# fugue-project/fugue

Hardware: NVIDIA H100
Metric: transform() rows/sec, hash-partitioned (num=256) identity map, 8-col table (higher is better)
Workload: dtype int64+f64 (byte moves; u64 hash arithmetic)

## Files before the change

### fugue_b200/csrc/fb_partition.cu

```cuda
#include <stdlib.h>

#include <mutex>

#include "fb_common.cuh"

namespace {

constexpr int kBlock = 512;
constexpr int kItems = 8;
constexpr int kTile = kBlock * kItems;
constexpr int kWarps = kBlock / 32;
constexpr int kCtasPerSm = 2;

struct FbCols {
  const void* src[FB_MAX_COLS];
  void* dst[FB_MAX_COLS];
  int32_t width[FB_MAX_COLS];
  int32_t ncols;
};

struct ChunkGeom {
  int64_t nrows;
  int64_t full_rows;
  int64_t tiles_per_chunk;
// ... 287 lines not shown
  while (c < cols.ncols) {
    T* __restrict__ buf = (T*)(cx.buf + (size_t)(phase & 1) * kTile);
#pragma unroll
    for (int r = 0; r < kItems; ++r) buf[pos[r]] = v[r];
    int nxt = c + 1;
    while (nxt < cols.ncols && cols.width[nxt] != (int)sizeof(T)) ++nxt;
    if (nxt < cols.ncols) load_col<T, kFull>(cols.src[nxt], warp_row0, warp_rows, lane, v);
    __syncthreads();
    T* __restrict__ out = (T*)cols.dst[c];
#pragma unroll
    for (int k = 0; k < kItems; ++k) {
      const int j = k * kBlock + (int)threadIdx.x;
      if (kFull || j < tile_rows) out[dst[k]] = buf[j];
    }
    ++phase;
    c = nxt;
  }
}

template <bool kSingleU64, int kBits, bool kFull, bool kAll8>
__device__ __forceinline__ void scatter_tile(const FbKeys& keys, const FbDiv& dv, const uint32_t num,
                                             const FbCols& cols, const TileCtx& cx,
                                             const int64_t tile_row0, const int tile_rows, int& phase) {
  const unsigned lane = threadIdx.x & 31, warp = threadIdx.x >> 5;
  const unsigned lt = fb_lanemask_lt();
  const uint32_t nb = num + 1;
  const uint32_t nbp = cx.nbp;
  uint32_t* __restrict__ my_cnt = cx.cnt + warp * nbp;
  const int64_t warp_row0 = tile_row0 + (int64_t)warp * (32 * kItems);
  const int warp_rows = tile_rows - (int)warp * (32 * kItems);

  uint32_t pid[kItems];
#pragma unroll
  for (int r = 0; r < kItems; ++r) {
    const bool ok = kFull || (r * 32 + (int)lane) < warp_rows;
    pid[r] = ok ? compute_pid<kSingleU64>(keys, dv, warp_row0 + r * 32 + lane) : num;
  }

  uint32_t pos[kItems];
#pragma unroll
  for (int r = 0; r < kItems; ++r) {
    const unsigned m = match_lanes<kBits + (kFull ? 0 : 1)>(pid[r], 0xFFFFFFFFu);
    const unsigned before = __popc(m & lt);
    uint32_t old = 0;
    if (before == 0) {
      old = my_cnt[pid[r]];
      my_cnt[pid[r]] = old + __popc(m);
    }
    __syncwarp();
    old = __shfl_sync(0xFFFFFFFFu, old, __ffs(m) - 1);
    pos[r] = old + before;
  }
  __syncthreads();

  {
    const uint32_t per = (nb + kBlock - 1) / kBlock;
    const uint32_t b0 = threadIdx.x * per;
    uint32_t tot[kMaxPer];
    uint32_t sum = 0;
#pragma unroll
    for (int i = 0; i < kMaxPer; ++i) {
      tot[i] = 0;
      if ((uint32_t)i < per && b0 + i < nb) {
        uint32_t run = 0;
#pragma unroll
        for (int w = 0; w < kWarps; ++w) {
          const uint32_t t = cx.cnt[w * nbp + b0 + i];
          cx.cnt[w * nbp + b0 + i] = run;
          run += t;
        }
        tot[i] = run;
        sum += run;
      }
    }
    uint32_t x = sum;
#pragma unroll
    for (int o = 1; o < 32; o <<= 1) {
      const uint32_t y = __shfl_up_sync(0xFFFFFFFFu, x, o);
      if (lane >= (unsigned)o) x += y;
    }
    if (lane == 31) cx.scanw[warp] = x;
    __syncthreads();
    uint32_t run = x - sum;
    {
      const uint32_t wt = lane < kWarps ? cx.scanw[lane] : 0;
#pragma unroll
      for (int w = 0; w < kWarps; ++w) {
        const uint32_t v = __shfl_sync(0xFFFFFFFFu, wt, w);
        if ((unsigned)w < warp) run += v;
      }
    }
#pragma unroll
    for (int i = 0; i < kMaxPer; ++i) {
      if ((uint32_t)i < per && b0 + i < nb) {
        const uint32_t cur = cx.cursor[b0 + i];
        cx.bin_start[b0 + i] = run;
        cx.delta[b0 + i] = cur - run;
        cx.cursor[b0 + i] = cur + tot[i];
        run += tot[i];
      }
    }
  }
  __syncthreads();

#pragma unroll
  for (int r = 0; r < kItems; ++r) {
    pos[r] += cx.bin_start[pid[r]] + my_cnt[pid[r]];
    cx.pid_sorted[pos[r]] = (uint16_t)pid[r];
  }
  __syncthreads();
  uint32_t dst[kItems];
#pragma unroll
  for (int k = 0; k < kItems; ++k) {
    const int j = k * kBlock + (int)threadIdx.x;
    dst[k] = cx.delta[cx.pid_sorted[j]] + (uint32_t)j;
  }
  for (uint32_t i = threadIdx.x; i < (uint32_t)kWarps * nbp; i += kBlock) cx.cnt[i] = 0;

  move_columns<uint64_t, kFull>(cols, cx, pos, dst, warp_row0, warp_rows, tile_rows, lane, phase);
  if (!kAll8) {
    move_columns<uint32_t, kFull>(cols, cx, pos, dst, warp_row0, warp_rows, tile_rows, lane, phase);
    move_columns<uint16_t, kFull>(cols, cx, pos, dst, warp_row0, warp_rows, tile_rows, lane, phase);
    move_columns<uint8_t, kFull>(cols, cx, pos, dst, warp_row0, warp_rows, tile_rows, lane, phase);
  }
  __syncthreads();
}

template <bool kSingleU64, int kBits, bool kAll8>
__global__ void __launch_bounds__(kBlock, kCtasPerSm)
fb_scatter_kernel(FbKeys keys, FbDiv dv, uint32_t num, ChunkGeom g, int chunk0,
                  const uint32_t* __restrict__ chunk_base, const int64_t* __restrict__ part_offsets,
                  FbCols cols) {
  extern __shared__ __align__(128) uint64_t smem64[];
  TileCtx cx;
  cx.nbp = nb_padded(num);
  cx.buf = smem64;
  cx.delta = (uint32_t*)(smem64 + 2 * kTile);
  cx.cursor = cx.delta + cx.nbp;
  cx.bin_start = cx.cursor + cx.nbp;
  cx.cnt = cx.bin_start + cx.nbp;
  cx.scanw = cx.cnt + kWarps * cx.nbp;
  cx.pid_sorted = (uint16_t*)(cx.scanw + 32);

  const int chunk = chunk0 + (int)blockIdx.x;
  int64_t chunk_row0, chunk_row1;
  chunk_range(g, chunk, chunk_row0, chunk_row1);

  for (uint32_t b = threadIdx.x; b < cx.nbp; b += kBlock)
    cx.cursor[b] = b < num ? (uint32_t)part_offsets[b] + chunk_base[(size_t)chunk * num + b] : 0u;
  for (uint32_t i = threadIdx.x; i < (uint32_t)kWarps * cx.nbp; i += kBlock) cx.cnt[i] = 0;
  __syncthreads();

  int phase = 0;
  for (int64_t tile_row0 = chunk_row0; tile_row0 < chunk_row1; tile_row0 += kTile) {
    const int64_t left = chunk_row1 - tile_row0;
    if (left >= kTile)
      scatter_tile<kSingleU64, kBits, true, kAll8>(keys, dv, num, cols, cx, tile_row0, kTile, phase);
    else
      scatter_tile<kSingleU64, kBits, false, kAll8>(keys, dv, num, cols, cx, tile_row0, (int)left, phase);
  }
}

constexpr int kSwcMaxCols = 8;
constexpr uint32_t kSwcMaxNum = 256;

__device__ __forceinline__ uint32_t smem_u32(const void* p) { return (uint32_t)__cvta_generic_to_shared(p); }

__device__ __forceinline__ void mbar_init(uint32_t bar, uint32_t count) {
  asm volatile("mbarrier.init.shared::cta.b64 [%0], %1;" ::"r"(bar), "r"(count) : "memory");
}
__device__ __forceinline__ void mbar_expect_tx(uint32_t bar, uint32_t bytes) {
  asm volatile("mbarrier.arrive.expect_tx.shared::cta.b64 _, [%0], %1;" ::"r"(bar), "r"(bytes) : "memory");
}
__device__ __forceinline__ void mbar_arrive_relaxed(uint32_t bar) {
  asm volatile("mbarrier.arrive.relaxed.cta.shared::cta.b64 _, [%0];" ::"r"(bar) : "memory");
}
__device__ __forceinline__ void mbar_wait(uint32_t bar, uint32_t parity) {
  asm volatile(
      "{\n"
      ".reg .pred p;\n"
      "FB_WAIT:\n"
      "mbarrier.try_wait.parity.shared::cta.b64 p, [%0], %1;\n"
      "@p bra FB_DONE;\n"
      "bra FB_WAIT;\n"
      "FB_DONE:\n"
      "}\n" ::"r"(bar), "r"(parity)
      : "memory");
}
__device__ __forceinline__ uint64_t l2_policy_evict_normal() {
  uint64_t pol;
  asm volatile("createpolicy.fractional.L2::evict_normal.b64 %0, 1.0;" : "=l"(pol));
  return pol;
}
__device__ __forceinline__ uint64_t l2_policy_evict_last() {
  uint64_t pol;
  asm volatile("createpolicy.fractional.L2::evict_last.b64 %0, 1.0;" : "=l"(pol));
  return pol;
}
__device__ __forceinline__ void tma_load_1d(uint32_t dst_smem, const void* src, uint32_t bytes, uint32_t bar,
                                            uint64_t policy) {
  asm volatile(
      "cp.async.bulk.shared::cluster.global.mbarrier::complete_tx::bytes.L2::cache_hint [%0], [%1], %2, [%3], %4;"
      ::"r"(dst_smem), "l"(src), "r"(bytes), "r"(bar), "l"(policy)
      : "memory");
}

constexpr int kWsMoverWarps = 16, kWsRankWarps = 8;
constexpr int kWsMovers = kWsMoverWarps * 32, kWsRankers = kWsRankWarps * 32;
constexpr int kWsThreads = kWsMovers + kWsRankers + 128;
constexpr int kWsG = 16;
constexpr int kWsGWide = 4;
constexpr int kWsMinStages = 3;
constexpr int kWsRankItems = 16;
constexpr uint32_t kWsProducerRegs = 24, kWsRankerRegs = 64, kWsMoverRegs = 88;
static_assert(128 * kWsProducerRegs + kWsRankers * kWsRankerRegs + kWsMovers * kWsMoverRegs <= kWsThreads * 72,
              "setmaxnreg: the roles take more registers than the launch gives the CTA");
constexpr int kMoveBatch = 8;

struct WsUnits {
  const uint64_t* src[FB_MAX_COLS];
  uint64_t* dst[FB_MAX_COLS];
  int32_t nunits;
  int32_t per_group;
  int32_t ngroups;
};

__device__ __forceinline__ void ws_chunk_run(const ChunkGeom& g, int i, int S, int& c0, int64_t& r0, int64_t& r1) {
  c0 = (int)((int64_t)i * g.nchunks_full / S);
  const int c1 = (int)((int64_t)(i + 1) * g.nchunks_full / S);
  int64_t unused;
  chunk_range(g, c0, r0, unused);
  chunk_range(g, c1 - 1, unused, r1);
}

struct WsMap {
  const uint64_t* src2[FB_MAX_COLS];
  uint64_t a[FB_MAX_COLS], b[FB_MAX_COLS], c[FB_MAX_COLS];
  int32_t mode[FB_MAX_COLS];
};

__device__ __forceinline__ uint64_t ws_apply_map(int mode, bool two, uint64_t x, uint64_t y, uint64_t a, uint64_t b,
                                                 uint64_t c) {
  if (mode == 1) {
    double r = __dmul_rn(__longlong_as_double((long long)a), __longlong_as_double((long long)x));
    if (two) r = __dadd_rn(r, __dmul_rn(__longlong_as_double((long long)b), __longlong_as_double((long long)y)));
    return (uint64_t)__double_as_longlong(__dadd_rn(r, __longlong_as_double((long long)c)));
  }
  if (mode == 2) return a * x + (two ? b * y : 0ULL) + c;
  return x;
}

template <int G, int RI>
__host__ __device__ inline size_t ws_book_bytes(uint32_t num, int ncols) {
  constexpr size_t kT = (size_t)kWsRankers * RI;
  const size_t nbp = nb_padded(num);
  const size_t E = (size_t)num * (G - 1);
  size_t b = 64 * 8;
  b += (size_t)ncols * E * 8;
  b += (kT + E) * 4;
  b += 5 * nbp * 4 + 64 * 4;
  b += ((E * 2 + 15) / 16) * 16;
  b += 2 * (size_t)kMetaBytes + 128;
  return b;
}

__device__ __forceinline__ void mbar_arrive(uint32_t bar) {
  asm volatile("mbarrier.arrive.shared::cta.b64 _, [%0];" ::"r"(bar) : "memory");
}
__device__ __forceinline__ void mover_sync() { asm volatile("bar.sync 1, %0;" ::"n"(kWsMovers) : "memory"); }
__device__ __forceinline__ void ranker_sync() { asm volatile("bar.sync 2, %0;" ::"n"(kWsRankers) : "memory"); }
template <uint32_t N>
__device__ __forceinline__ void setmaxnreg_dec() { asm volatile("setmaxnreg.dec.sync.aligned.u32 %0;" ::"n"(N)); }
template <uint32_t N>
__device__ __forceinline__ void setmaxnreg_inc() { asm volatile("setmaxnreg.inc.sync.aligned.u32 %0;" ::"n"(N)); }

template <int kBits, int G, int kWsRankItems, bool kMap>
__global__ void __launch_bounds__(kWsThreads, 1)
fb_scatter_ws_kernel(WsUnits units, uint32_t num, ChunkGeom g, int nstages,
                     const uint8_t* __restrict__ meta,
                     const uint32_t* __restrict__ chunk_base, const int64_t* __restrict__ part_offsets,
                     const __grid_constant__ WsMap map) {
  constexpr uint32_t T = (uint32_t)kWsRankers * kWsRankItems;
  static_assert(T == (uint32_t)kTile, "pass 1 ranks tiles of kTile rows");
  static_assert(G >= 2 && G <= 16 && (G & (G - 1)) == 0, "G must be a power of two <= 16");
  constexpr uint32_t GM = G - 1;
  constexpr uint32_t kStageBytes = T * 8;
  constexpr int kSlotRounds = ((int)T + (int)kSwcMaxNum * (G - 1) + kWsMovers - 1) / kWsMovers;
  constexpr int kEntryRoundsM = ((int)kSwcMaxNum * (G - 1) + kWsMovers - 1) / kWsMovers;
  extern __shared__ __align__(128) uint64_t smem64[];
  const uint32_t nbp = nb_padded(num);
  const uint32_t E = num * GM;
  const int grp = (int)blockIdx.x % units.ngroups;
  int chunk0;
  int64_t row0, row1;
  ws_chunk_run(g, (int)blockIdx.x / units.ngroups, (int)gridDim.x / units.ngroups, chunk0, row0, row1);
  const int u0 = grp * units.per_group;
  const int ncols = min(units.per_group, units.nunits - u0);
  uint64_t* ring = smem64;
  uint64_t* bars = ring + (size_t)nstages * T;
  uint64_t* carry = bars + 64;
  uint32_t* slotinfo = (uint32_t*)(carry + (size_t)ncols * E);
  uint32_t* wpos = slotinfo + T + E;
  uint32_t* kcnt = wpos + nbp;
  uint32_t* binfo = kcnt + nbp;
  uint32_t* wstart = binfo + nbp;
  uint32_t* wdelta = wstart + nbp;
  uint32_t* scanw = wdelta + nbp;
  uint16_t* carryinfo = (uint16_t*)(scanw + 64);
  uint8_t* metabuf = (uint8_t*)(((uintptr_t)(carryinfo + E) + 127) & ~(uintptr_t)127);

  const unsigned lane = threadIdx.x & 31, warp = threadIdx.x >> 5;
  const uint32_t bar_full = smem_u32(bars), bar_empty = smem_u32(bars + 16);
  const uint32_t bar_pid_full = smem_u32(bars + 32), bar_pid_empty = smem_u32(bars + 34);
  const uint32_t bar_slots_ready = smem_u32(bars + 36), bar_slots_free = smem_u32(bars + 37);

  if (threadIdx.x == 0) {
    for (int s = 0; s < nstages; ++s) {
      mbar_init(bar_full + 8 * s, 1);
      mbar_init(bar_empty + 8 * s, kWsMoverWarps);
    }
    for (int i = 0; i < 2; ++i) {
      mbar_init(bar_pid_full + 8 * i, 1);
      mbar_init(bar_pid_empty + 8 * i, kWsRankWarps);
    }
    mbar_init(bar_slots_ready, kWsRankWarps);
    mbar_init(bar_slots_free, kWsMoverWarps);
    asm volatile("fence.mbarrier_init.release.cluster;" ::: "memory");
  }
  __syncthreads();

  if (warp >= kWsMoverWarps + kWsRankWarps) {
    setmaxnreg_dec<kWsProducerRegs>();
    if (warp == kWsMoverWarps + kWsRankWarps && lane == 0) {
      const uint64_t pol = l2_policy_evict_normal(), meta_pol = l2_policy_evict_last();
      const uint32_t ring_s = smem_u32(ring), meta_s = smem_u32(metabuf);
      uint32_t s = 0, ph = 0, seq = 0;
      auto load_pid = [&](int64_t t, uint32_t q) {
        const uint32_t b = q & 1, pp = (q >> 1) & 1;
        mbar_wait(bar_pid_empty + 8 * b, pp ^ 1);
        mbar_expect_tx(bar_pid_full + 8 * b, kMetaBytes);
        tma_load_1d(meta_s + b * kMetaBytes, meta + (size_t)(t / T) * kMetaBytes, kMetaBytes,
                    bar_pid_full + 8 * b, meta_pol);
      };
      load_pid(row0, 0);
      for (int64_t t0 = row0; t0 < row1; t0 += T, ++seq) {
        if (t0 + T < row1) load_pid(t0 + T, seq + 1);
        for (int u = u0; u < u0 + ncols; ++u) {
          mbar_wait(bar_empty + 8 * s, ph ^ 1);
          mbar_expect_tx(bar_full + 8 * s, kStageBytes);
          tma_load_1d(ring_s + s * kStageBytes, units.src[u] + t0, kStageBytes, bar_full + 8 * s, pol);
          if (++s == (uint32_t)nstages) { s = 0; ph ^= 1; }
          if constexpr (kMap) {
            if (map.src2[u] != nullptr) {
              mbar_wait(bar_empty + 8 * s, ph ^ 1);
              mbar_expect_tx(bar_full + 8 * s, kStageBytes);
              tma_load_1d(ring_s + s * kStageBytes, map.src2[u] + t0, kStageBytes, bar_full + 8 * s, pol);
              if (++s == (uint32_t)nstages) { s = 0; ph ^= 1; }
            }
          }
        }
      }
    }
    return;
  }

  if (warp >= kWsMoverWarps) {
    setmaxnreg_dec<kWsRankerRegs>();
    const unsigned rw = warp - kWsMoverWarps;
    const unsigned rtid = threadIdx.x - kWsMovers;
    for (uint32_t b = rtid; b < nbp; b += kWsRankers) {
      const uint32_t p0 = b < num ? (uint32_t)part_offsets[b] + chunk_base[(size_t)chunk0 * num + b] : 0u;
      wpos[b] = p0 & ~GM;
      kcnt[b] = (p0 & GM) | ((p0 & GM) << 8);
    }
    ranker_sync();
    uint32_t seq = 0;
    for (int64_t t0 = row0; t0 < row1; t0 += T, ++seq) {
      const uint32_t pb = seq & 1, pph = (seq >> 1) & 1;
      mbar_wait(bar_pid_full + 8 * pb, pph);
      const uint8_t* __restrict__ rec = metabuf + pb * kMetaBytes;
      const uint32_t b = rtid;
      uint32_t n = 0, w = 0, kold = 0, phold = 0, wp_old = 0;
      if (b < num) n = ((const uint16_t*)(rec + kMetaCnt))[b];
      if (b < num) {
        const uint32_t kc = kcnt[b];
        kold = kc & 0xFFu;
        phold = kc >> 8;
        wp_old = wpos[b];
        const uint32_t end = wp_old + kold + n;
        const uint32_t aend = end & ~GM;
        if (aend > wp_old) {
          w = aend - wp_old;
          wpos[b] = aend;
          kcnt[b] = end - aend;
        } else {
          kcnt[b] = (kold + n) | (phold << 8);
        }
        binfo[b] = kold | (w << 8);
      }
      uint32_t xw = w;
#pragma unroll
      for (int o = 1; o < 32; o <<= 1) {
        const uint32_t yw = __shfl_up_sync(0xFFFFFFFFu, xw, o);
        if (lane >= (unsigned)o) xw += yw;
      }
      if (lane == 31) scanw[8 + rw] = xw;
      ranker_sync();
      uint32_t bw = xw - w;
      {
        const uint32_t tw = lane < kWsRankWarps ? scanw[8 + lane] : 0;
#pragma unroll
        for (int wi = 0; wi < kWsRankWarps; ++wi) {
          const uint32_t vw = __shfl_sync(0xFFFFFFFFu, tw, wi);
          if ((unsigned)wi < rw) bw += vw;
        }
      }
      if (seq > 0) mbar_wait(bar_slots_free, (seq - 1) & 1);
      if (b < num) {
        wstart[b] = bw;
        wdelta[b] = wp_old - bw;
      }
      if (rtid == kWsRankers - 1) scanw[40] = bw + w;
      ranker_sync();
#pragma unroll
      for (int r = 0; r < kWsRankItems; ++r) {
        const uint32_t row = r * kWsRankers + rtid;
        const uint32_t pb2 = rec[row];
        const uint32_t bi = binfo[pb2];
        const uint32_t i = (bi & 0xFFu) + ((const uint16_t*)(rec + kMetaRank))[row];
        const uint32_t ww = bi >> 8;
        if (i < ww) slotinfo[wstart[pb2] + i] = (pb2 << 16) | row;
        else carryinfo[pb2 * GM + (i - ww)] = (uint16_t)row;
      }
      __syncwarp();
      if (lane == 0) mbar_arrive_relaxed(bar_pid_empty + 8 * pb);
      if (b < num) {
#pragma unroll
        for (uint32_t i = 0; i < GM; ++i) {
          const uint32_t e = b * GM + i;
          const uint32_t desc = i < phold ? 0xFFFFu : T + e;
          if (i < kold) {
            if (i < w) slotinfo[bw + i] = (b << 16) | desc;
            else carryinfo[e] = (uint16_t)desc;
          }
          if (w + i >= kold + n) carryinfo[e] = 0xFFFFu;
        }
      }
      ranker_sync();
      if (lane == 0) mbar_arrive(bar_slots_ready);
    }
    return;
  }

  setmaxnreg_inc<kWsMoverRegs>();
  uint32_t s = 0, ph = 0, seq = 0;
  for (int64_t t0 = row0; t0 < row1; t0 += T, ++seq) {
    mbar_wait(bar_slots_ready, seq & 1);
    const uint32_t W = scanw[40];
    uint32_t srcd[kSlotRounds], dst[kSlotRounds];
#pragma unroll
    for (int k = 0; k < kSlotRounds; ++k) {
      const uint32_t j = k * kWsMovers + threadIdx.x;
      srcd[k] = 0xFFFFu;
      dst[k] = 0;
      if (j < W) {
        const uint32_t info = slotinfo[j];
        srcd[k] = info & 0xFFFFu;
        dst[k] = wdelta[info >> 16] + j;
      }
    }
    uint32_t csrc[kEntryRoundsM];
#pragma unroll
    for (int q = 0; q < kEntryRoundsM; ++q) {
      const uint32_t e = q * kWsMovers + threadIdx.x;
      const uint32_t d = e < E ? (uint32_t)carryinfo[e] : 0xFFFFu;
      csrc[q] = d < T ? d : 0xFFFFu;
    }
    __syncwarp();
    if (lane == 0) mbar_arrive(bar_slots_free);

    for (int u = 0; u < ncols; ++u) {
      mbar_wait(bar_full + 8 * s, ph);
      const uint64_t* __restrict__ st = ring + (size_t)s * T;
      uint64_t* __restrict__ out = units.dst[u0 + u];
      uint64_t* __restrict__ cbuf = carry + (size_t)u * E;
      uint32_t s2 = s;
      bool two = false;
      const uint64_t* __restrict__ st2 = st;
      int mode = 0;
      uint64_t ma = 0, mb = 0, mc = 0;
      if constexpr (kMap) {
        mode = map.mode[u0 + u];
        two = map.src2[u0 + u] != nullptr;
        if (two) {
          s2 = s + 1 == (uint32_t)nstages ? 0 : s + 1;
          mbar_wait(bar_full + 8 * s2, s2 == 0 ? ph ^ 1 : ph);
          st2 = ring + (size_t)s2 * T;
        }
        ma = map.a[u0 + u]; mb = map.b[u0 + u]; mc = map.c[u0 + u];
      }
      auto staged = [&](uint32_t r) -> uint64_t {
        if constexpr (kMap) return ws_apply_map(mode, two, st[r], st2[r], ma, mb, mc);
        else return st[r];
      };
#pragma unroll
      for (int k0 = 0; k0 < kSlotRounds; k0 += kMoveBatch) {
        uint64_t v[kMoveBatch];
#pragma unroll
        for (int k = 0; k < kMoveBatch; ++k)
          if (k0 + k < kSlotRounds && srcd[k0 + k] != 0xFFFFu)
            v[k] = srcd[k0 + k] < T ? staged(srcd[k0 + k]) : cbuf[srcd[k0 + k] - T];
#pragma unroll
        for (int k = 0; k < kMoveBatch; ++k)
          if (k0 + k < kSlotRounds && srcd[k0 + k] != 0xFFFFu) out[dst[k0 + k]] = v[k];
      }
      mover_sync();
#pragma unroll
      for (int q = 0; q < kEntryRoundsM; ++q)
        if (csrc[q] != 0xFFFFu) cbuf[q * kWsMovers + threadIdx.x] = staged(csrc[q]);
      __syncwarp();
      if (lane == 0) {
        mbar_arrive_relaxed(bar_empty + 8 * s);
        if (kMap && two) mbar_arrive_relaxed(bar_empty + 8 * s2);
      }
      if (++s == (uint32_t)nstages) { s = 0; ph ^= 1; }
      if (kMap && two) {
        if (++s == (uint32_t)nstages) { s = 0; ph ^= 1; }
      }
    }
    if (ncols == 1) mover_sync();
  }
  mover_sync();
  for (int u = 0; u < ncols; ++u) {
    uint64_t* __restrict__ out = units.dst[u0 + u];
    const uint64_t* __restrict__ cbuf = carry + (size_t)u * E;
#pragma unroll
    for (int q = 0; q < kEntryRoundsM; ++q) {
      const uint32_t e = q * kWsMovers + threadIdx.x;
      if (e < E) {
        const uint32_t b = e / GM, i = e - b * GM;
        const uint32_t kc = kcnt[b];
        if (i < (kc & 0xFFu) && i >= (kc >> 8)) out[wpos[b] + i] = cbuf[e];
      }
    }
  }
}

__global__ void fb_bits_to_bytes_kernel(const uint8_t* __restrict__ bits, int64_t bit_offset,
                                        int64_t nrows, uint8_t* __restrict__ out) {
  int64_t i = (int64_t)blockIdx.x * blockDim.x + threadIdx.x;
  int64_t stride = (int64_t)gridDim.x * blockDim.x;
  for (; i < nrows; i += stride) {
    int64_t j = i + bit_offset;
    out[i] = (bits[j >> 3] >> (j & 7)) & 1;
  }
}

__global__ void fb_bytes_to_bits_kernel(const uint8_t* __restrict__ bytes, int64_t nrows,
                                        uint8_t* __restrict__ out, unsigned long long* null_count) {
  int64_t nbytes = (nrows + 7) >> 3;
  int64_t i = (int64_t)blockIdx.x * blockDim.x + threadIdx.x;
  int64_t stride = (int64_t)gridDim.x * blockDim.x;
  unsigned long long nulls = 0;
  for (; i < nbytes; i += stride) {
    uint8_t v = 0;
#pragma unroll
    for (int k = 0; k < 8; ++k) {
      int64_t r = i * 8 + k;
      if (r < nrows) {
        if (bytes[r]) v |= (uint8_t)(1u << k);
        else ++nulls;
      }
    }
    out[i] = v;
  }
  if (null_count != nullptr && nulls) atomicAdd(null_count, nulls);
}

inline int bits_for(uint32_t num) { return num <= 16 ? 4 : (num <= 256 ? 8 : 10); }

#define FB_DISPATCH_SB(single, bits, LAUNCH)                 \
  do {                                                       \
    if (single) {                                            \
      if (bits == 4) LAUNCH(true, 4);                        \
      else if (bits == 8) LAUNCH(true, 8);                   \
      else LAUNCH(true, 10);                                 \
    } else {                                                 \
      if (bits == 4) LAUNCH(false, 4);                       \
      else if (bits == 8) LAUNCH(false, 8);                  \
      else LAUNCH(false, 10);                                \
    }                                                        \
  } while (0)

template <typename K>
cudaError_t optin(K kernel, size_t bytes) {
  return cudaFuncSetAttribute(kernel, cudaFuncAttributeMaxDynamicSharedMemorySize, (int)bytes);
}

cudaError_t ensure_smem_optin(int dev) {
  static std::mutex mu;
  static uint64_t done = 0;
  std::lock_guard<std::mutex> lock(mu);
  if (dev >= 0 && dev < 64 && (done >> dev) & 1) return cudaSuccess;
  const size_t sc = scatter_smem_bytes(FB_MAX_PARTITIONS);
  const size_t hs = (size_t)kHistWarps * FB_MAX_PARTITIONS * sizeof(uint32_t);
  cudaError_t e = cudaSuccess;
#define FB_OPTIN(S, B)                                                   \
  do {                                                                   \
    if (e == cudaSuccess) e = optin(fb_scatter_kernel<S, B, true>, sc);  \
    if (e == cudaSuccess) e = optin(fb_scatter_kernel<S, B, false>, sc); \
    if (e == cudaSuccess) e = optin(fb_hist_kernel<S, B>, hs);           \
  } while (0)
  {
    int smem_max = 0;
    if (e == cudaSuccess) e = cudaDeviceGetAttribute(&smem_max, cudaDevAttrMaxSharedMemoryPerBlockOptin, dev);
#define FB_OPTIN_WS(G)                                                                                        \
  do {                                                                                                        \
    if (e == cudaSuccess) e = optin(fb_scatter_ws_kernel<4, G, kWsRankItems, false>, (size_t)smem_max);       \
    if (e == cudaSuccess) e = optin(fb_scatter_ws_kernel<8, G, kWsRankItems, false>, (size_t)smem_max);       \
    if (e == cudaSuccess) e = optin(fb_scatter_ws_kernel<4, G, kWsRankItems, true>, (size_t)smem_max);        \
    if (e == cudaSuccess) e = optin(fb_scatter_ws_kernel<8, G, kWsRankItems, true>, (size_t)smem_max);        \
  } while (0)
    FB_OPTIN_WS(kWsG);
    FB_OPTIN_WS(kWsGWide);
#undef FB_OPTIN_WS
  }
  FB_OPTIN(true, 4); FB_OPTIN(true, 8); FB_OPTIN(true, 10);
  FB_OPTIN(false, 4); FB_OPTIN(false, 8); FB_OPTIN(false, 10);
#undef FB_OPTIN
  if (e == cudaSuccess && dev >= 0 && dev < 64) done |= (1ull << dev);
  return e;
}

bool single_u64_key(int nkeys, const int32_t* widths, const uint8_t* const* valid) {
  return nkeys == 1 && widths[0] == 8 && (valid == nullptr || valid[0] == nullptr);
}

int fill_keys(FbKeys& k, int nkeys, const void* const* ptrs, const int32_t* widths,
              const uint8_t* const* valid) {
  FB_CHECK(nkeys >= 1 && nkeys <= FB_MAX_KEYS, "nkeys=%d out of range [1,%d]", nkeys, FB_MAX_KEYS);
  memset(&k, 0, sizeof(k));
  k.nkeys = nkeys;
  k.digit_shift = -1;
  for (int i = 0; i < nkeys; ++i) {
    FB_CHECK(widths[i] == 1 || widths[i] == 2 || widths[i] == 4 || widths[i] == 8,
             "key %d has unsupported width %d", i, widths[i]);
    FB_CHECK(ptrs[i] != nullptr, "key %d pointer is NULL", i);
    k.ptr[i] = ptrs[i];
    k.width[i] = widths[i];
    k.valid[i] = valid ? valid[i] : nullptr;
  }
  return 0;
}

struct PlanLayout {
  size_t hist_bytes;
  size_t pid_offset;
  size_t total_bytes;
};

PlanLayout plan_layout(const ChunkGeom& g, uint32_t num) {
  PlanLayout l;
  l.hist_bytes = (((size_t)g.nchunks * num * sizeof(uint32_t)) + 255) & ~(size_t)255;
  l.pid_offset = l.hist_bytes + 256;
  l.total_bytes = l.pid_offset + (num <= kSwcMaxNum ? (size_t)(g.full_rows / kTile) * kMetaBytes : 0) + 256;
  return l;
}

}

extern "C" {

size_t fb_partition_scratch_bytes(int dev, int64_t nrows, uint32_t num_partitions) {
  if (nrows < 0 || num_partitions == 0) return 0;
  ChunkGeom g = make_geom(dev, nrows);
  return plan_layout(g, num_partitions).total_bytes;
}

int fb_partition_ids(int dev, void* stream, int64_t nrows, int nkeys, const void* const* key_ptrs,
                     const int32_t* key_widths, const uint8_t* const* key_valid,
                     uint32_t num_partitions, uint32_t* out_pids) {
  FB_CHECK(nrows >= 0, "nrows < 0");
  FB_CHECK(num_partitions >= 1, "num_partitions must be >= 1");
  if (nrows == 0) return 0;
  FbDeviceGuard guard(dev);
  FB_CHECK(guard.ok, "cannot select device %d", dev);
  FbKeys k;
  if (int rc = fill_keys(k, nkeys, key_ptrs, key_widths, key_valid)) return rc;
  FbDiv dv = fb_make_div(num_partitions);
  int64_t blocks = (nrows + 255) / 256;
  int64_t maxb = (int64_t)fb_sm_count(dev) * 16;
  if (blocks > maxb) blocks = maxb;
  cudaStream_t st = (cudaStream_t)stream;
  if (single_u64_key(nkeys, key_widths, key_valid))
    fb_pid_kernel<true><<<(unsigned)blocks, 256, 0, st>>>(k, dv, nrows, out_pids);
  else
    fb_pid_kernel<false><<<(unsigned)blocks, 256, 0, st>>>(k, dv, nrows, out_pids);
  FB_CUDA(cudaGetLastError());
  return 0;
}

int fb_row_hash64(int dev, void* stream, int64_t nrows, int nkeys, const void* const* key_ptrs,
                  const int32_t* key_widths, const uint8_t* const* key_valid, uint64_t* out_hash) {
  FB_CHECK(nrows >= 0, "nrows < 0");
  if (nrows == 0) return 0;
  FbDeviceGuard guard(dev);
  FB_CHECK(guard.ok, "cannot select device %d", dev);
  FbKeys k;
  if (int rc = fill_keys(k, nkeys, key_ptrs, key_widths, key_valid)) return rc;
  int64_t blocks = (nrows + 255) / 256;
  int64_t maxb = (int64_t)fb_sm_count(dev) * 16;
  if (blocks > maxb) blocks = maxb;
  fb_row_hash_kernel<<<(unsigned)blocks, 256, 0, (cudaStream_t)stream>>>(k, nrows, out_hash);
  FB_CUDA(cudaGetLastError());
  return 0;
}

static int plan_impl(int dev, void* stream, int64_t nrows, const FbKeys& k, bool single,
                     uint32_t num_partitions, void* scratch, size_t scratch_bytes,
                     int64_t* out_part_offsets) {
  FB_CHECK(nrows >= 0, "nrows < 0");
  FB_CHECK(nrows < ((int64_t)1 << 32), "nrows=%lld exceeds the 2^32-1 rows one call handles",
           (long long)nrows);
  FB_CHECK(num_partitions >= 1 && num_partitions <= FB_MAX_PARTITIONS,
           "num_partitions=%u out of range [1,%d]", num_partitions, FB_MAX_PARTITIONS);
  FB_CHECK(out_part_offsets != nullptr, "out_part_offsets is NULL");
  FbDeviceGuard guard(dev);
  FB_CHECK(guard.ok, "cannot select device %d", dev);
  cudaStream_t st = (cudaStream_t)stream;
  if (nrows == 0) {
    FB_CUDA(cudaMemsetAsync(out_part_offsets, 0, sizeof(int64_t) * ((size_t)num_partitions + 1), st));
    return 0;
  }
  ChunkGeom g = make_geom(dev, nrows);
  PlanLayout l = plan_layout(g, num_partitions);
  FB_CHECK(scratch != nullptr && scratch_bytes >= l.total_bytes,
           "scratch too small: need %zu bytes, got %zu", l.total_bytes, scratch_bytes);
  FbDiv dv = fb_make_div(num_partitions);
  uint32_t* hist = (uint32_t*)scratch;
  size_t smem = (size_t)kHistWarps * num_partitions * sizeof(uint32_t);
  FB_CUDA(ensure_smem_optin(dev));
  const int bits = bits_for(num_partitions);
  int hist_chunk0 = 0;
  if (num_partitions <= kSwcMaxNum && g.nchunks_full > 0) {
    uint8_t* meta = (uint8_t*)scratch + l.pid_offset;
#define FB_LAUNCH_RANK(S, B, STAGED) \
  fb_rank_tile_kernel<S, B, STAGED><<<g.nchunks_full, kRankBlock, 0, st>>>(k, dv, num_partitions, g, hist, meta)
    if (single) {
      if (bits == 4) FB_LAUNCH_RANK(true, 4, true);
      else FB_LAUNCH_RANK(true, 8, true);
    } else if (k.digit_shift >= 0) {
// ... 335 lines not shown
```

Baseline: 18.61 billion.

## Streamline ranker slot assignment with packed per-bucket info and fewer barriers

Bucket metadata (carry count, write width, intra-warp prefix) is packed into one double-buffered word per bucket. This removes the separate binfo/wstart arrays and one named-barrier round per tile. Each ranker thread now reads the ids and ranks of 16 contiguous rows as 128-bit vector loads instead of strided byte and halfword loads. The cross-warp offset comes from a shuffle scan and a per-partition shuffle. The carry-fill logic is rewritten to touch only the needed entries and ends with a warp sync rather than a full ranker barrier. This relies on the field widths (4-bit carry, 13-bit width) and on every row's slot write seeing the other warps' pin entries after the single remaining barrier. The changed row-to-thread mapping also alters slot order, which risks subtle races or incorrect bookkeeping.

```diff
diff --git a/fugue_b200/csrc/fb_partition.cu b/fugue_b200/csrc/fb_partition.cu
--- a/fugue_b200/csrc/fb_partition.cu
+++ b/fugue_b200/csrc/fb_partition.cu
@@ -613,9 +613,8 @@
   uint32_t* slotinfo = (uint32_t*)(carry + (size_t)ncols * E);
   uint32_t* wpos = slotinfo + T + E;
   uint32_t* kcnt = wpos + nbp;
-  uint32_t* binfo = kcnt + nbp;
-  uint32_t* wstart = binfo + nbp;
-  uint32_t* wdelta = wstart + nbp;
+  uint32_t* pinfo = kcnt + nbp;
+  uint32_t* wdelta = pinfo + 2 * nbp;
   uint32_t* scanw = wdelta + nbp;
   uint16_t* carryinfo = (uint16_t*)(scanw + 64);
   uint8_t* metabuf = (uint8_t*)(((uintptr_t)(carryinfo + E) + 127) & ~(uintptr_t)127);
@@ -684,12 +683,15 @@
       wpos[b] = p0 & ~GM;
       kcnt[b] = (p0 & GM) | ((p0 & GM) << 8);
     }
+    for (uint32_t e = rtid; e < E; e += kWsRankers) carryinfo[e] = 0xFFFFu;
     ranker_sync();
+    static_assert(kWsRankItems == 16, "a ranker thread reads the ids and ranks of its 16 rows as 128-bit words");
     uint32_t seq = 0;
     for (int64_t t0 = row0; t0 < row1; t0 += T, ++seq) {
       const uint32_t pb = seq & 1, pph = (seq >> 1) & 1;
       mbar_wait(bar_pid_full + 8 * pb, pph);
       const uint8_t* __restrict__ rec = metabuf + pb * kMetaBytes;
+      uint32_t* __restrict__ pin = pinfo + pb * nbp;
       const uint32_t b = rtid;
       uint32_t n = 0, w = 0, kold = 0, phold = 0, wp_old = 0;
       if (b < num) n = ((const uint16_t*)(rec + kMetaCnt))[b];
@@ -707,7 +709,6 @@
         } else {
           kcnt[b] = (kold + n) | (phold << 8);
         }
-        binfo[b] = kold | (w << 8);
       }
       uint32_t xw = w;
 #pragma unroll
@@ -715,49 +716,53 @@
         const uint32_t yw = __shfl_up_sync(0xFFFFFFFFu, xw, o);
         if (lane >= (unsigned)o) xw += yw;
       }
-      if (lane == 31) scanw[8 + rw] = xw;
+      if (b < num) pin[b] = kold | (w << 4) | ((xw - w) << 17);
+      if (lane == 31) scanw[8 * pb + rw] = xw;
       ranker_sync();
-      uint32_t bw = xw - w;
+      uint32_t woff = lane < kWsRankWarps ? scanw[8 * pb + lane] : 0;
+      uint32_t W;
       {
-        const uint32_t tw = lane < kWsRankWarps ? scanw[8 + lane] : 0;
-#pragma unroll
-        for (int wi = 0; wi < kWsRankWarps; ++wi) {
-          const uint32_t vw = __shfl_sync(0xFFFFFFFFu, tw, wi);
-          if ((unsigned)wi < rw) bw += vw;
+        uint32_t x = woff;
+#pragma unroll
+        for (int o = 1; o < kWsRankWarps; o <<= 1) {
+          const uint32_t y = __shfl_up_sync(0xFFFFFFFFu, x, o);
+          if (lane >= (unsigned)o) x += y;
         }
-      }
+        woff = x - woff;
+        W = __shfl_sync(0xFFFFFFFFu, x, kWsRankWarps - 1);
+      }
+      const uint32_t bw = xw - w + __shfl_sync(0xFFFFFFFFu, woff, rw);
       if (seq > 0) mbar_wait(bar_slots_free, (seq - 1) & 1);
-      if (b < num) {
-        wstart[b] = bw;
-        wdelta[b] = wp_old - bw;
-      }
-      if (rtid == kWsRankers - 1) scanw[40] = bw + w;
-      ranker_sync();
+      if (b < num) wdelta[b] = wp_old - bw;
+      if (rtid == 0) scanw[40] = W;
+      const uint32_t r0 = rtid * kWsRankItems;
+      const uint4 idw = *(const uint4*)(rec + r0);
+      const uint4 rk0 = *(const uint4*)(rec + kMetaRank + 2 * r0);
+      const uint4 rk1 = *(const uint4*)(rec + kMetaRank + 2 * r0 + 16);
+      const uint32_t ids[4] = {idw.x, idw.y, idw.z, idw.w};
+      const uint32_t rks[8] = {rk0.x, rk0.y, rk0.z, rk0.w, rk1.x, rk1.y, rk1.z, rk1.w};
+      uint32_t inf[kWsRankItems];
+#pragma unroll
+      for (int r = 0; r < kWsRankItems; ++r) inf[r] = pin[(ids[r >> 2] >> (8 * (r & 3))) & 0xFFu];
 #pragma unroll
       for (int r = 0; r < kWsRankItems; ++r) {
-        const uint32_t row = r * kWsRankers + rtid;
-        const uint32_t pb2 = rec[row];
-        const uint32_t bi = binfo[pb2];
-        const uint32_t i = (bi & 0xFFu) + ((const uint16_t*)(rec + kMetaRank))[row];
-        const uint32_t ww = bi >> 8;
-        if (i < ww) slotinfo[wstart[pb2] + i] = (pb2 << 16) | row;
-        else carryinfo[pb2 * GM + (i - ww)] = (uint16_t)row;
+        const uint32_t p = (ids[r >> 2] >> (8 * (r & 3))) & 0xFFu;
+        const uint32_t i = (inf[r] & 0xFu) + ((rks[r >> 1] >> (16 * (r & 1))) & 0xFFFFu);
+        const uint32_t ww = (inf[r] >> 4) & 0x1FFFu;
+        const uint32_t slot0 = (inf[r] >> 17) + __shfl_sync(0xFFFFFFFFu, woff, p >> 5);
+        if (i < ww) slotinfo[slot0 + i] = (p << 16) | (r0 + r);
+        else carryinfo[p * GM + (i - ww)] = (uint16_t)(r0 + r);
       }
       __syncwarp();
       if (lane == 0) mbar_arrive_relaxed(bar_pid_empty + 8 * pb);
       if (b < num) {
-#pragma unroll
-        for (uint32_t i = 0; i < GM; ++i) {
-          const uint32_t e = b * GM + i;
-          const uint32_t desc = i < phold ? 0xFFFFu : T + e;
-          if (i < kold) {
-            if (i < w) slotinfo[bw + i] = (b << 16) | desc;
-            else carryinfo[e] = (uint16_t)desc;
-          }
-          if (w + i >= kold + n) carryinfo[e] = 0xFFFFu;
+        const uint32_t c = kold + n - w;
+        if (w > 0) {
+          for (uint32_t i = 0; i < kold; ++i) slotinfo[bw + i] = (b << 16) | (i < phold ? 0xFFFFu : T + b * GM + i);
         }
-      }
-      ranker_sync();
+        for (uint32_t i = w > 0 ? c : 0; i < kold; ++i) carryinfo[b * GM + i] = 0xFFFFu;
+      }
+      __syncwarp();
       if (lane == 0) mbar_arrive(bar_slots_ready);
     }
     return;
```

After: 18.65 billion, median of 6. About the same (+0.2%).
